# zhu-xlab/PFST

Measured on AMD Instinct MI355X. Metric: PFST train-step images/s on 1024² IRRG tiles, higher is better.
Workload: dtype f32 (f16x3 split MFMA: two scaled fp16 pieces per operand, three products, fp32 accumulate); 1 GPU; pfst_pots_irrg2vaih_irrg_deeplabv3plus_r50-d8; global_batch=8, per_gpu_batch=8, tile=1024x1024x3, num_classes=6, parallelism=dp1, weights=seeded random init, conv_math=f16x3

## Files before the change

### pfst_amd/csrc/conv_winograd.hip

```cpp
#include "common.h"
#include "amax.h"
#include "weight_jobs.h"

namespace {

template <int M> struct Wino;
template <> struct Wino<2> {
  static constexpr int R = 4;
  static constexpr float bt(int i, int j) {
    constexpr float m[4][4] = {{1, 0, -1, 0}, {0, 1, 1, 0}, {0, -1, 1, 0}, {0, 1, 0, -1}};
    return m[i][j];
  }
  static constexpr float g(int i, int j) {
    constexpr float m[4][3] = {{1, 0, 0}, {.5f, .5f, .5f}, {.5f, -.5f, .5f}, {0, 0, 1}};
    return m[i][j];
  }
  static constexpr float at(int i, int j) {
    constexpr float m[2][4] = {{1, 1, 1, 0}, {0, 1, -1, -1}};
    return m[i][j];
  }
};
template <> struct Wino<4> {
  static constexpr int R = 6;
  static constexpr float bt(int i, int j) {
    constexpr float m[6][6] = {{4, 0, -5, 0, 1, 0}, {0, -4, -4, 1, 1, 0}, {0, 4, -4, -1, 1, 0},
                               {0, -2, -1, 2, 1, 0}, {0, 2, -1, -2, 1, 0}, {0, 4, 0, -5, 0, 1}};
    return m[i][j];
  }
  static constexpr float g(int i, int j) {
    constexpr float m[6][3] = {{1.f / 4, 0, 0}, {-1.f / 6, -1.f / 6, -1.f / 6}, {-1.f / 6, 1.f / 6, -1.f / 6},
                               {1.f / 24, 1.f / 12, 1.f / 6}, {1.f / 24, -1.f / 12, 1.f / 6}, {0, 0, 1}};
    return m[i][j];
  }
  static constexpr float at(int i, int j) {
    constexpr float m[4][6] = {{1, 1, 1, 1, 1, 0}, {0, 1, -1, 2, -2, 0}, {0, 1, 1, 4, 4, 0}, {0, 1, -1, 8, -8, 1}};
    return m[i][j];
  }
};
__device__ __forceinline__ float cmac(float acc, float coef, float v) {
  if (coef == 0.f) return acc;
  if (coef == 1.f) return acc + v;
  if (coef == -1.f) return acc - v;
  return fmaf(coef, v, acc);
}

struct WinoGeom {
  int H, W, d, Hs, Ws, Th, Tw, T;
};
inline WinoGeom wino_geom(int H, int W, int d, int m) {
  WinoGeom g;
  g.H = H; g.W = W; g.d = d;
  g.Hs = (H + d - 1) / d; g.Ws = (W + d - 1) / d;
  g.Th = (g.Hs + m - 1) / m; g.Tw = (g.Ws + m - 1) / m;
  g.T = d * d * g.Th * g.Tw;
  return g;
}
__device__ __forceinline__ void tile_coord(const WinoGeom& g, int t, int& sy, int& sx, int& ty, int& tx) {
  sx = t % g.d; t /= g.d;
  tx = t % g.Tw; t /= g.Tw;
  ty = t % g.Th;
  sy = t / g.Th;
}

template <int M>
__device__ __forceinline__ void filter_tf(const float (&g)[3][3], float (&u)[M + 2][M + 2]) {
  constexpr int R = M + 2;
  float t[R][3];
#pragma unroll
  for (int i = 0; i < R; ++i)
#pragma unroll
    for (int j = 0; j < 3; ++j) {
      float a = 0.f;
#pragma unroll
      for (int k = 0; k < 3; ++k) a = cmac(a, Wino<M>::g(i, k), g[k][j]);
      t[i][j] = a;
    }
#pragma unroll
  for (int i = 0; i < R; ++i)
#pragma unroll
    for (int j = 0; j < R; ++j) {
      float a = 0.f;
#pragma unroll
      for (int k = 0; k < 3; ++k) a = cmac(a, Wino<M>::g(j, k), t[i][k]);
      u[i][j] = a;
    }
}
template <int M, bool PLAIN>
__global__ void wino_filter_kernel(const float* __restrict__ w, float* __restrict__ Uf, float* __restrict__ Ud, int Cout, int Cin) {
  constexpr int R = M + 2;
  const i64 total = (i64)Cout * Cin;
  for (i64 i = (i64)blockIdx.x * blockDim.x + threadIdx.x; i < total; i += (i64)gridDim.x * blockDim.x) {
    const int ci = (int)(i % Cin), co = (int)(i / Cin);
    float g[3][3], gf[3][3], u[R][R];
#pragma unroll
    for (int a = 0; a < 3; ++a)
#pragma unroll
      for (int b = 0; b < 3; ++b) {
        g[a][b] = w[i * 9 + a * 3 + b];
        gf[2 - a][2 - b] = g[a][b];
      }
    if (Uf) {
      filter_tf<M>(g, u);
      const i64 at = PLAIN ? i : ((i64)(ci >> 2) * Cout + co) * 4 + (ci & 3);
#pragma unroll
      for (int xi = 0; xi < R * R; ++xi) Uf[(i64)xi * total + at] = u[xi / R][xi % R];
    }
    if (Ud) {
      filter_tf<M>(gf, u);
      const i64 at = PLAIN ? i : ((i64)(co >> 2) * Cin + ci) * 4 + (co & 3);
#pragma unroll
      for (int xi = 0; xi < R * R; ++xi) Ud[(i64)xi * total + at] = u[xi / R][xi % R];
    }
  }
}

template <int M>
__global__ __launch_bounds__(256) void wino_input_kernel(const float* __restrict__ x, i64 x_bs, float* __restrict__ V, int N, int C,
                                                         WinoGeom g, int vec, float* __restrict__ amax, const float* __restrict__ pack_amax,
                                                         int pack_shift, const float4* __restrict__ bnl) {
  float am = 0.f;
  float ps = 0.f;
  if (pack_amax) {
    int e = amax_exponent(amax_read(pack_amax)) + pack_shift;
    e = e > 254 ? 254 : e;
    ps = scale_of(e);
    if (amax && blockIdx.x == 0 && blockIdx.y == 0 && blockIdx.z == 0 && threadIdx.x == 0) amax[0] = __builtin_bit_cast(float, (unsigned)e << 23);
  }
  constexpr int R = M + 2;
  typedef float vecM __attribute__((ext_vector_type(M)));
  const int c = blockIdx.y, n = blockIdx.z;
  const float* xp = x + (i64)n * x_bs + (i64)c * g.H * g.W;
  const i64 plane = (i64)N * C * g.T;
  float* vp = V + ((i64)n * C + c) * g.T;
  float nsc = 1.f, nsh = 0.f;
  if (bnl) {
    const float4 cf = bnl[c];
    nsc = cf.z;
    nsh = cf.w;
  }
  auto norm = [&](float v, bool in) { return bnl ? (in ? fmaxf(__fmaf_rn(v, nsc, nsh), 0.f) : 0.f) : v; };
  for (int t = blockIdx.x * blockDim.x + threadIdx.x; t < g.T; t += gridDim.x * blockDim.x) {
    int sy, sx, ty, tx;
    tile_coord(g, t, sy, sx, ty, tx);
    float d[R][R];
    if (vec) {
      const int x0 = M * tx;
#pragma unroll
      for (int a = 0; a < R; ++a) {
        const int y = M * ty - 1 + a;
        const bool in = y >= 0 && y < g.H;
        const float* row = xp + (i64)y * g.W + x0;
        vecM mid;
#pragma unroll
        for (int b = 0; b < M; ++b) mid[b] = 0.f;
        if (in) mid = *reinterpret_cast<const vecM*>(row);
        const bool inl = in && x0 > 0, inr = in && x0 + M < g.W;
        d[a][0] = norm(inl ? row[-1] : 0.f, inl);
#pragma unroll
        for (int b = 0; b < M; ++b) d[a][1 + b] = norm(mid[b], in);
        d[a][R - 1] = norm(inr ? row[M] : 0.f, inr);
      }
    } else {
#pragma unroll
      for (int a = 0; a < R; ++a) {
        const int y = sy + g.d * (M * ty - 1 + a);
#pragma unroll
        for (int b = 0; b < R; ++b) {
          const int xx = sx + g.d * (M * tx - 1 + b);
          const bool in = y >= 0 && y < g.H && xx >= 0 && xx < g.W;
          d[a][b] = norm(in ? xp[(i64)y * g.W + xx] : 0.f, in);
        }
      }
    }
    float r[R][R];
#pragma unroll
    for (int i = 0; i < R; ++i)
#pragma unroll
      for (int b = 0; b < R; ++b) {
        float a = 0.f;
#pragma unroll
        for (int k = 0; k < R; ++k) a = cmac(a, Wino<M>::bt(i, k), d[k][b]);
        r[i][b] = a;
      }
#pragma unroll
    for (int i = 0; i < R; ++i)
#pragma unroll
      for (int j = 0; j < R; ++j) {
        float a = 0.f;
#pragma unroll
        for (int k = 0; k < R; ++k) a = cmac(a, Wino<M>::bt(j, k), r[i][k]);
        if (pack_amax) {
          reinterpret_cast<unsigned*>(vp)[(i64)(i * R + j) * plane + t] = pack_f16x2_pieces(a * ps);
        } else {
          vp[(i64)(i * R + j) * plane + t] = a;
          am = fmaxf(am, fabsf(a));
        }
      }
  }
  if (amax && !pack_amax) amax_publish(amax, am);
}

template <int M>
__global__ __launch_bounds__(256) void wino_output_kernel(const float* __restrict__ Mb, float* __restrict__ y, i64 y_bs, int N, int Cout,
                                                          WinoGeom g, int accumulate, int vec, float* __restrict__ stats, int stats_minmax,
                                                          const float* __restrict__ bnb_x, i64 bnb_x_bs, const float4* __restrict__ bnb_coef, int bnb_relu) {
  constexpr int R = M + 2;
  typedef float vecM __attribute__((ext_vector_type(M)));
  __shared__ double red[32];
  float st_s = 0.f, st_q = 0.f;
  float st_lo = __builtin_inff(), st_hi = -__builtin_inff();
  const int c = blockIdx.y, n = blockIdx.z;
  float* yp = y + (i64)n * y_bs + (i64)c * g.H * g.W;
  const float* bxp = bnb_x ? bnb_x + (i64)n * bnb_x_bs + (i64)c * g.H * g.W : nullptr;
  const float bsc = bnb_x ? bnb_coef[c].z : 0.f, bsh = bnb_x ? bnb_coef[c].w : 0.f;
  const i64 plane = (i64)N * Cout * g.T;
  const float* mp = Mb + ((i64)n * Cout + c) * g.T;
  for (int t = blockIdx.x * blockDim.x + threadIdx.x; t < g.T; t += gridDim.x * blockDim.x) {
    int sy, sx, ty, tx;
    tile_coord(g, t, sy, sx, ty, tx);
    float m[R][R];
#pragma unroll
    for (int i = 0; i < R * R; ++i) m[i / R][i % R] = __builtin_nontemporal_load(&mp[(i64)i * plane + t]);
    float r[M][R];
#pragma unroll
    for (int i = 0; i < M; ++i)
#pragma unroll
      for (int b = 0; b < R; ++b) {
        float a = 0.f;
#pragma unroll
        for (int k = 0; k < R; ++k) a = cmac(a, Wino<M>::at(i, k), m[k][b]);
        r[i][b] = a;
      }
#pragma unroll
    for (int i = 0; i < M; ++i) {
      const int yy = sy + g.d * (M * ty + i);
      if (yy >= g.H) continue;
      float o[M];
#pragma unroll
      for (int j = 0; j < M; ++j) {
        float a = 0.f;
#pragma unroll
        for (int k = 0; k < R; ++k) a = cmac(a, Wino<M>::at(j, k), r[i][k]);
        o[j] = a;
      }
      const int x0 = sx + g.d * (M * tx);
      if (vec) {
        vecM* q = reinterpret_cast<vecM*>(yp + (i64)yy * g.W + x0);
        vecM v;
#pragma unroll
        for (int j = 0; j < M; ++j) v[j] = o[j];
        if (accumulate) v += *q;
        *q = v;
        if (bxp) {
          const vecM xv = *reinterpret_cast<const vecM*>(bxp + (i64)yy * g.W + x0);
#pragma unroll
          for (int j = 0; j < M; ++j) {
            const float dz = (!bnb_relu || __fmaf_rn(xv[j], bsc, bsh) > 0.f) ? v[j] : 0.f;
            st_s += dz;
            st_q = fmaf(dz, xv[j], st_q);
          }
          continue;
        }
#pragma unroll
        for (int j = 0; j < M; ++j) {
          const float e = v[j];
          st_s += e;
          st_q = fmaf(e, e, st_q);
          st_lo = fminf(st_lo, e);
          st_hi = fmaxf(st_hi, e);
        }
        continue;
      }
#pragma unroll
      for (int j = 0; j < M; ++j) {
        const int xx = x0 + g.d * j;
        if (xx < g.W) {
          float* q = yp + (i64)yy * g.W + xx;
          const float v = accumulate ? *q + o[j] : o[j];
          *q = v;
          if (bxp) {
            const float xs = bxp[(i64)yy * g.W + xx];
            const float dz = (!bnb_relu || __fmaf_rn(xs, bsc, bsh) > 0.f) ? v : 0.f;
            st_s += dz;
            st_q = fmaf(dz, xs, st_q);
          } else {
            st_s += v;
            st_q = fmaf(v, v, st_q);
            st_lo = fminf(st_lo, v);
            st_hi = fmaxf(st_hi, v);
          }
        }
      }
    }
  }
  if (stats) {
    double bs = (double)st_s, bq = (double)st_q;
    block_sum2_d<true>(bs, bq, red);
    if (threadIdx.x == 0) {
      const i64 T = (i64)gridDim.x * gridDim.z;
      float2* dst = reinterpret_cast<float2*>(stats) + ((i64)c * T + (i64)n * gridDim.x + blockIdx.x);
      *dst = make_float2((float)bs, (float)bq);
    }
    if (stats_minmax) {
#pragma unroll
      for (int o = 32; o > 0; o >>= 1) {
        st_lo = fminf(st_lo, __shfl_xor(st_lo, o));
        st_hi = fmaxf(st_hi, __shfl_xor(st_hi, o));
      }
      float* mm = reinterpret_cast<float*>(red);
      __syncthreads();
      if ((threadIdx.x & 63) == 0) { mm[threadIdx.x >> 6] = st_lo; mm[8 + (threadIdx.x >> 6)] = st_hi; }
      __syncthreads();
      if (threadIdx.x == 0) {
        const int nw = (blockDim.x + 63) >> 6;
        for (int i = 1; i < nw; ++i) { st_lo = fminf(st_lo, mm[i]); st_hi = fmaxf(st_hi, mm[8 + i]); }
        const i64 T = (i64)gridDim.x * gridDim.z;
        float2* dst = reinterpret_cast<float2*>(stats) + ((i64)Cout * T + (i64)c * T + (i64)n * gridDim.x + blockIdx.x);
        *dst = make_float2(st_lo, st_hi);
      }
    }
  }
}

template <int M>
__global__ __launch_bounds__(256) void wino_dy_kernel(const float* __restrict__ dy, i64 dy_bs, float* __restrict__ dM, int N, int Cout,
                                                      WinoGeom g, float* __restrict__ amax, const float* __restrict__ pack_amax, int pack_shift) {
  float am = 0.f;
  float ps = 0.f;
  if (pack_amax) {
    int e = amax_exponent(amax_read(pack_amax)) + pack_shift;
    e = e > 254 ? 254 : e;
    ps = scale_of(e);
    if (amax && blockIdx.x == 0 && blockIdx.y == 0 && blockIdx.z == 0 && threadIdx.x == 0) amax[0] = __builtin_bit_cast(float, (unsigned)e << 23);
  }
  constexpr int R = M + 2;
  const int c = blockIdx.y, n = blockIdx.z;
  const float* gp = dy + (i64)n * dy_bs + (i64)c * g.H * g.W;
  const i64 plane = (i64)N * Cout * g.T;
  float* mp = dM + ((i64)n * Cout + c) * g.T;
  for (int t = blockIdx.x * blockDim.x + threadIdx.x; t < g.T; t += gridDim.x * blockDim.x) {
    int sy, sx, ty, tx;
    tile_coord(g, t, sy, sx, ty, tx);
    float e[M][M];
#pragma unroll
    for (int i = 0; i < M; ++i)
#pragma unroll
      for (int j = 0; j < M; ++j) {
        const int yy = sy + g.d * (M * ty + i), xx = sx + g.d * (M * tx + j);
        e[i][j] = (yy < g.H && xx < g.W) ? gp[(i64)yy * g.W + xx] : 0.f;
      }
    float r[R][M];
#pragma unroll
    for (int a = 0; a < R; ++a)
#pragma unroll
      for (int j = 0; j < M; ++j) {
        float s = 0.f;
#pragma unroll
        for (int i = 0; i < M; ++i) s = cmac(s, Wino<M>::at(i, a), e[i][j]);
        r[a][j] = s;
      }
#pragma unroll
    for (int a = 0; a < R; ++a)
#pragma unroll
      for (int b = 0; b < R; ++b) {
        float s = 0.f;
#pragma unroll
        for (int j = 0; j < M; ++j) s = cmac(s, Wino<M>::at(j, b), r[a][j]);
        if (pack_amax) {
          reinterpret_cast<unsigned*>(mp)[(i64)(a * R + b) * plane + t] = pack_f16x2_pieces(s * ps);
        } else {
          mp[(i64)(a * R + b) * plane + t] = s;
          am = fmaxf(am, fabsf(s));
        }
      }
  }
  if (amax && !pack_amax) amax_publish(amax, am);
}

template <int M>
__global__ void wino_dw_kernel(const float* __restrict__ dU, float* __restrict__ dw, int Cout, int Cin) {
  constexpr int R = M + 2;
  const i64 total = (i64)Cout * Cin;
  for (i64 i = (i64)blockIdx.x * blockDim.x + threadIdx.x; i < total; i += (i64)gridDim.x * blockDim.x) {
    float u[R][R];
#pragma unroll
    for (int xi = 0; xi < R * R; ++xi) u[xi / R][xi % R] = dU[(i64)xi * total + i];
    float t[3][R];
#pragma unroll
    for (int p = 0; p < 3; ++p)
#pragma unroll
      for (int b = 0; b < R; ++b) {
        float s = 0.f;
#pragma unroll
        for (int a = 0; a < R; ++a) s = cmac(s, Wino<M>::g(a, p), u[a][b]);
        t[p][b] = s;
      }
#pragma unroll
    for (int p = 0; p < 3; ++p)
#pragma unroll
      for (int q = 0; q < 3; ++q) {
        float s = 0.f;
#pragma unroll
        for (int b = 0; b < R; ++b) s = cmac(s, Wino<M>::g(b, q), t[p][b]);
        dw[i * 9 + p * 3 + q] += s;
      }
  }
}

template <int M>
__device__ __forceinline__ void weight_prep_wino(const pfst_weight_job_t& J, int lb, float (*red)[36]) {
  constexpr int R = M + 2, X = R * R;
  const i64 total = (i64)J.Cout * J.Cin;
  const i64 i = (i64)lb * 256 + threadIdx.x;
  const bool live = i < total;
  float g[3][3], gf[3][3], u[R][R];
#pragma unroll
  for (int a = 0; a < 3; ++a)
#pragma unroll
    for (int b = 0; b < 3; ++b) {
      g[a][b] = live ? J.src[i * 9 + a * 3 + b] : 0.f;
      gf[2 - a][2 - b] = g[a][b];
    }
#pragma unroll
  for (int dir = 0; dir < 2; ++dir) {
    float* dst = reinterpret_cast<float*>(dir ? J.dst_d : J.dst_f);
    float* amax = dir ? J.amax_d : J.amax_f;
    if (!dst) continue;
    filter_tf<M>(dir ? gf : g, u);
#pragma unroll
    for (int xi = 0; xi < X; ++xi) {
      const float v = u[xi / R][xi % R];
      if (live) dst[(i64)xi * total + i] = v;
      float m = fabsf(v);
#pragma unroll
      for (int o = 32; o > 0; o >>= 1) m = fmaxf(m, __shfl_xor(m, o));
      if ((threadIdx.x & 63) == 0) red[threadIdx.x >> 6][xi] = m;
    }
    __syncthreads();
    if (threadIdx.x < X) {
      const float m = fmaxf(fmaxf(red[0][threadIdx.x], red[1][threadIdx.x]), fmaxf(red[2][threadIdx.x], red[3][threadIdx.x]));
      if (m > 0.f)
        atomicMax(reinterpret_cast<unsigned*>(amax) + (i64)threadIdx.x * PFST_AMAX_SUB + (lb & (PFST_AMAX_SUB - 1)), __builtin_bit_cast(unsigned, m));
    }
    __syncthreads();
  }
}

__global__ __launch_bounds__(256) void weight_prep_batched_kernel(const pfst_weight_job_t* __restrict__ jobs, int njobs) {
  __shared__ float red[4][36];
  const pfst_weight_job_t J = jobs[weight_job_of_block(jobs, njobs, blockIdx.x)];
  const int lb = blockIdx.x - J.first_block;
  if (J.m == 2) return weight_prep_wino<2>(J, lb, red);
  if (J.m == 4) return weight_prep_wino<4>(J, lb, red);
  const i64 n = (i64)J.Cout * J.Cin * J.T;
  float m = 0.f;
#pragma unroll 4
  for (int k = 0; k < 16; ++k) {
    const i64 i = (i64)lb * 4096 + k * 256 + threadIdx.x;
    if (i < n) m = fmaxf(m, fabsf(J.src[i]));
  }
#pragma unroll
  for (int o = 32; o > 0; o >>= 1) m = fmaxf(m, __shfl_xor(m, o));
  if ((threadIdx.x & 63) == 0) red[threadIdx.x >> 6][0] = m;
  __syncthreads();
  if (threadIdx.x == 0) {
    m = fmaxf(fmaxf(red[0][0], red[1][0]), fmaxf(red[2][0], red[3][0]));
    if (m > 0.f) atomicMax(reinterpret_cast<unsigned*>(J.amax_f) + (lb & (PFST_AMAX_SUB - 1)), __builtin_bit_cast(unsigned, m));
  }
}

inline int tile_blocks(int T) {
  int b = (T + 255) / 256;
  return b < 1 ? 1 : b;
}

#define PFST_WINO_M(m_, CALL2, CALL4) \
  do {                                \
    if ((m_) == 2) { CALL2; } else { CALL4; } \
  } while (0)

}

#define PFST_CHECK_TILE(m) PFST_CHECK_ARG((m) == 2 || (m) == 4)

extern "C" int pfst_wino_tiles(int H, int W, int dil, int m) {
  if (H <= 0 || W <= 0 || dil < 1 || (m != 2 && m != 4)) return 0;
  return wino_geom(H, W, dil, m).T;
}

extern "C" int pfst_wino_pack_weight(const float* w, float* U_fprop, float* U_dgrad, int Cout, int Cin, int m, pfst_stream_t stream) {
  PFST_CHECK_ARG(w && (U_fprop || U_dgrad) && Cout > 0 && Cin > 0);
  PFST_CHECK_TILE(m);
  PFST_CHECK_ARG((!U_fprop || Cin % 16 == 0) && (!U_dgrad || Cout % 16 == 0));
  const dim3 grid(ew_grid((i64)Cout * Cin));
  PFST_WINO_M(m, hipLaunchKernelGGL((wino_filter_kernel<2, false>), grid, dim3(256), 0, (hipStream_t)stream, w, U_fprop, U_dgrad, Cout, Cin),
              hipLaunchKernelGGL((wino_filter_kernel<4, false>), grid, dim3(256), 0, (hipStream_t)stream, w, U_fprop, U_dgrad, Cout, Cin));
  PFST_CHECK_LAUNCH();
  return PFST_OK;
}

extern "C" int pfst_wino_filter_plain(const float* w, float* P_fprop, float* P_dgrad, int Cout, int Cin, int m, pfst_stream_t stream) {
  PFST_CHECK_ARG(w && (P_fprop || P_dgrad) && Cout > 0 && Cin > 0);
  PFST_CHECK_TILE(m);
  const dim3 grid(ew_grid((i64)Cout * Cin));
  PFST_WINO_M(m, hipLaunchKernelGGL((wino_filter_kernel<2, true>), grid, dim3(256), 0, (hipStream_t)stream, w, P_fprop, P_dgrad, Cout, Cin),
              hipLaunchKernelGGL((wino_filter_kernel<4, true>), grid, dim3(256), 0, (hipStream_t)stream, w, P_fprop, P_dgrad, Cout, Cin));
  PFST_CHECK_LAUNCH();
  return PFST_OK;
}

extern "C" int pfst_weight_job_blocks(const pfst_weight_job_t* job, int pack) { return job ? weight_job_blocks(*job, pack) : 0; }

extern "C" int pfst_weight_prep_batched(const pfst_weight_job_t* jobs_host, const pfst_weight_job_t* jobs_dev, int njobs, pfst_stream_t stream) {
  PFST_CHECK_ARG(jobs_host && jobs_dev && njobs > 0);
  i64 blocks = 0;
  for (int j = 0; j < njobs; ++j) {
    const pfst_weight_job_t& J = jobs_host[j];
    PFST_CHECK_ARG(J.src && J.Cout > 0 && J.Cin > 0 && (J.m == 0 || J.m == 2 || J.m == 4) && J.first_block == blocks);
    if (J.m == 0) PFST_CHECK_ARG(J.amax_f && (J.T == 1 || J.T == 9));
    else PFST_CHECK_ARG(J.T == 9 && (J.dst_f || J.dst_d) && (!J.dst_f || J.amax_f) && (!J.dst_d || J.amax_d));
    blocks += weight_job_blocks(J, 0);
  }
  PFST_CHECK_ARG(blocks < (1ll << 31));
  hipLaunchKernelGGL(weight_prep_batched_kernel, dim3((unsigned)blocks), dim3(256), 0, (hipStream_t)stream, jobs_dev, njobs);
  PFST_CHECK_LAUNCH();
  return PFST_OK;
}

extern "C" int pfst_wino_input(const float* x, long long x_bs, float* V, int N, int C, int H, int W, int dil, int m, float* v_amax,
                               const float* pack_x_amax, const float* bnl, pfst_stream_t stream) {
  PFST_CHECK_ARG(!pack_x_amax || v_amax);
  PFST_CHECK_ARG(!bnl || ((uintptr_t)bnl & 15) == 0);
  const int shift_in = m == 4 ? 7 : 3;
  PFST_CHECK_ARG(x && V && N > 0 && N <= 65535 && C > 0 && C <= 65535 && H > 0 && W > 0 && dil >= 1 && x_bs >= (i64)C * H * W);
  PFST_CHECK_TILE(m);
  const WinoGeom g = wino_geom(H, W, dil, m);
  const int vec = dil == 1 && W % m == 0 && x_bs % m == 0 && ((uintptr_t)x & (4 * m - 1)) == 0;
  const dim3 grid(tile_blocks(g.T), C, N);
  PFST_WINO_M(m, hipLaunchKernelGGL(wino_input_kernel<2>, grid, dim3(256), 0, (hipStream_t)stream, x, x_bs, V, N, C, g, vec, v_amax, pack_x_amax, shift_in, (const float4*)bnl),
              hipLaunchKernelGGL(wino_input_kernel<4>, grid, dim3(256), 0, (hipStream_t)stream, x, x_bs, V, N, C, g, vec, v_amax, pack_x_amax, shift_in, (const float4*)bnl));
  PFST_CHECK_LAUNCH();
  return PFST_OK;
}

extern "C" int pfst_wino_gemm(const float* V, const float* U, float* Mbuf, int N, int K, int M, int T, int m, pfst_stream_t stream) {
  PFST_CHECK_ARG(V && U && Mbuf && N > 0 && N <= 65535 && K > 0 && K % 16 == 0 && M > 0 && T > 0);
  PFST_CHECK_TILE(m);
  PFST_CHECK_ARG((i64)K * T * 4 < (1ll << 31) && (i64)M * T * 4 < (1ll << 31) && (i64)K * M * 4 < (1ll << 31));
  return pfst_igemm_q_launch(V, (i64)K * T, U, nullptr, Mbuf, (i64)M * T, N, K, 1, T, M, 1, T, 1, 1, 1, 0, 1, 0, nullptr, 0,
                             (m + 2) * (m + 2), (hipStream_t)stream);
}

extern "C" int pfst_wino_stats_slots(int H, int W, int dil, int m) {
  if (H <= 0 || W <= 0 || dil < 1 || (m != 2 && m != 4)) return 0;
  return tile_blocks(wino_geom(H, W, dil, m).T);
}

extern "C" int pfst_wino_output(const float* Mbuf, float* y, long long y_bs, int N, int Cout, int H, int W, int dil, int accumulate,
                                float* stats, int stats_minmax, const float* bnb_x, long long bnb_x_bs, const float* bnb_coef, int bnb_relu, int m,
                                pfst_stream_t stream) {
  PFST_CHECK_ARG(Mbuf && y && N > 0 && N <= 65535 && Cout > 0 && Cout <= 65535 && H > 0 && W > 0 && dil >= 1 && y_bs >= (i64)Cout * H * W);
  PFST_CHECK_ARG(!stats_minmax || stats);
  PFST_CHECK_ARG(!bnb_x || (stats && !stats_minmax && bnb_coef && bnb_x_bs >= (i64)Cout * H * W && (bnb_x_bs % 4) == 0 && ((uintptr_t)bnb_x & 15) == 0));
  PFST_CHECK_TILE(m);
  const WinoGeom g = wino_geom(H, W, dil, m);
  const int vec = dil == 1 && W % m == 0 && y_bs % m == 0 && ((uintptr_t)y & (4 * m - 1)) == 0;
  const dim3 grid(tile_blocks(g.T), Cout, N);
  PFST_WINO_M(m, hipLaunchKernelGGL(wino_output_kernel<2>, grid, dim3(256), 0, (hipStream_t)stream, Mbuf, y, y_bs, N, Cout, g, accumulate, vec, stats, stats_minmax, bnb_x,
                                 (i64)bnb_x_bs, reinterpret_cast<const float4*>(bnb_coef), bnb_relu),
              hipLaunchKernelGGL(wino_output_kernel<4>, grid, dim3(256), 0, (hipStream_t)stream, Mbuf, y, y_bs, N, Cout, g, accumulate, vec, stats, stats_minmax, bnb_x,
                                 (i64)bnb_x_bs, reinterpret_cast<const float4*>(bnb_coef), bnb_relu));
  PFST_CHECK_LAUNCH();
  return PFST_OK;
}

extern "C" int pfst_wino_dy(const float* dy, long long dy_bs, float* dM, int N, int Cout, int H, int W, int dil, int m, float* dm_amax,
                            const float* pack_dy_amax, pfst_stream_t stream) {
  PFST_CHECK_ARG(!pack_dy_amax || dm_amax);
  const int shift_dy = m == 4 ? 8 : 2;
  PFST_CHECK_ARG(dy && dM && N > 0 && N <= 65535 && Cout > 0 && Cout <= 65535 && H > 0 && W > 0 && dil >= 1 && dy_bs >= (i64)Cout * H * W);
  PFST_CHECK_TILE(m);
  const WinoGeom g = wino_geom(H, W, dil, m);
  const dim3 grid(tile_blocks(g.T), Cout, N);
  PFST_WINO_M(m, hipLaunchKernelGGL(wino_dy_kernel<2>, grid, dim3(256), 0, (hipStream_t)stream, dy, dy_bs, dM, N, Cout, g, dm_amax, pack_dy_amax, shift_dy),
              hipLaunchKernelGGL(wino_dy_kernel<4>, grid, dim3(256), 0, (hipStream_t)stream, dy, dy_bs, dM, N, Cout, g, dm_amax, pack_dy_amax, shift_dy));
  PFST_CHECK_LAUNCH();
  return PFST_OK;
}

extern "C" int pfst_wino_wgrad(const float* V, const float* dM, float* dU, float* dw, int N, int Cin, int Cout, int T, int m,
                               int split, const float* v_amax, const float* dm_amax, int packed, pfst_stream_t stream) {
  PFST_CHECK_ARG(V && dM && dU && dw && N > 0 && N <= 65535 && Cin > 0 && Cout > 0 && T > 0 && T % 4 == 0);
  PFST_CHECK_ARG(split != 2 || (v_amax && dm_amax && Cout > 64));
  PFST_CHECK_ARG(!packed || split == 2);
  PFST_CHECK_TILE(m);
  hipStream_t s = (hipStream_t)stream;
  const i64 uc = (i64)Cout * Cin;
  const int nx = (m + 2) * (m + 2);
  if (hipMemsetAsync(dU, 0, nx * uc * sizeof(float), s) != hipSuccess) return PFST_ERR_LAUNCH;
  const int rc = split == 2 ? pfst_wgrad_f16x3_launch(V, (i64)Cin * T, dM, (i64)Cout * T, dU, N, Cin, Cout, T, nx, (i64)N * Cin * T,
                                                      (i64)N * Cout * T, uc, v_amax, dm_amax, packed, s)
                 : split ? pfst_wgrad_split_q_launch(V, (i64)Cin * T, dM, (i64)Cout * T, dU, N, Cin, Cout, T, nx, (i64)N * Cin * T,
                                                   (i64)N * Cout * T, uc, s)
                       : pfst_wgrad_q_launch(V, (i64)Cin * T, dM, (i64)Cout * T, dU, N, Cin, 1, T, Cout, 1, T, 1, 1, 0, nx, (i64)N * Cin * T,
                                             (i64)N * Cout * T, uc, s);
  if (rc != PFST_OK) return rc;
  PFST_WINO_M(m, hipLaunchKernelGGL(wino_dw_kernel<2>, dim3(ew_grid(uc)), dim3(256), 0, s, dU, dw, Cout, Cin),
              hipLaunchKernelGGL(wino_dw_kernel<4>, dim3(ew_grid(uc)), dim3(256), 0, s, dU, dw, Cout, Cin));
  PFST_CHECK_LAUNCH();
  return PFST_OK;
}
```

Baseline: 29.59 images/s.

## Stage Winograd input/dy/output row bands through LDS with coalesced vector loads

Adds an LDS staging path for the Winograd input, dy and output transform kernels. Each 256-thread block loads or stores its contiguous band of image rows with coalesced float4 accesses into padded shared memory, where wino_pos adds bank-conflict padding. Tiles are then read from or written to LDS instead of through strided global gathers, which matters most for dilated convolutions. The cost is up to 63KB of dynamic LDS per block, which can lower occupancy, plus extra barriers and more template variants. The path can be disabled with the PFST_WINO_STAGED environment variable, and the output kernel uses it only when dilation is greater than 1.

Measured after the change: 29.83 images/s (median of 6 runs). About the same (+0.8%).

```diff
diff --git a/pfst_amd/csrc/conv_winograd.hip b/pfst_amd/csrc/conv_winograd.hip
--- a/pfst_amd/csrc/conv_winograd.hip
+++ b/pfst_amd/csrc/conv_winograd.hip
@@ -1,3 +1,4 @@
+#include <stdlib.h>
 #include "common.h"
 #include "amax.h"
 #include "weight_jobs.h"
@@ -62,6 +63,105 @@
   sy = t / g.Th;
 }
 
+typedef float f4 __attribute__((ext_vector_type(4)));
+constexpr int kWinoStageBudget = 63 * 1024;
+struct WinoStage {
+  int on, LP, XE, P, rows;
+};
+__host__ __device__ __forceinline__ int wino_pos(int x, int d) { return x + d * (x >> 5); }
+inline WinoStage wino_stage(const WinoGeom& g, int m, int halo, int images, bool aligned, unsigned& bytes) {
+  WinoStage st = {0, 0, 0, 0, 0};
+  bytes = 0;
+  const char* e = getenv("PFST_WINO_STAGED");
+  if ((e && e[0] == '0' && !e[1]) || !aligned || g.W % 4 != 0 || (halo && g.d > 4)) return st;
+  const i64 L = (i64)g.Tw * g.d;
+  i64 nty = 256 % L == 0 ? 256 / L : 254 / L + 2;
+  nty = nty > g.Th ? g.Th : nty;
+  st.LP = halo ? 4 : 0;
+  st.XE = g.d * m * g.Tw + (halo ? g.d : 0);
+  st.P = (wino_pos(st.LP + st.XE - 1, g.d) + 1) | 1;
+  st.rows = (int)(m * nty + 2 * halo);
+  const i64 need = (i64)images * st.rows * st.P * 4;
+  if (need > kWinoStageBudget) return st;
+  bytes = (unsigned)need;
+  st.on = 1;
+  return st;
+}
+__device__ __forceinline__ int div_u(int a, int b, float rb) {
+  int q = (int)((float)a * rb);
+  const int r = a - q * b;
+  q += (r >= b) - (r < 0);
+  return q;
+}
+struct WinoBand {
+  int ok, sy, ty0, nty, tbase, L;
+  float rL, rd;
+};
+__device__ __forceinline__ WinoBand wino_band(const WinoGeom& g, const WinoStage& st, int m, int halo) {
+  WinoBand b;
+  const int t0 = blockIdx.x * 256, t1 = min(t0 + 255, g.T - 1);
+  int sx, tx, sy1, ty1;
+  tile_coord(g, t0, b.sy, sx, b.ty0, tx);
+  tile_coord(g, t1, sy1, sx, ty1, tx);
+  b.nty = ty1 - b.ty0 + 1;
+  b.L = g.Tw * g.d;
+  b.tbase = (b.sy * g.Th + b.ty0) * b.L;
+  b.ok = st.on && sy1 == b.sy && m * b.nty + 2 * halo <= st.rows;
+  b.rL = 1.f / (float)b.L;
+  b.rd = 1.f / (float)g.d;
+  return b;
+}
+__device__ __forceinline__ void band_coord(const WinoGeom& g, const WinoBand& b, int t, int& tyr, int& sx, int& tx) {
+  const int rel = t - b.tbase;
+  tyr = div_u(rel, b.L, b.rL);
+  const int rem = rel - tyr * b.L;
+  tx = div_u(rem, g.d, b.rd);
+  sx = rem - tx * g.d;
+}
+template <bool PADS, bool NT>
+__device__ __forceinline__ void stage_rows(float* __restrict__ lds, const float* __restrict__ src, const WinoGeom& g, const WinoStage& st, int sy,
+                                           int r0, int NR, bool norm, float nsc, float nsh) {
+  const int W4 = g.W >> 2, n4 = NR * W4;
+  const float rW4 = 1.f / (float)W4;
+  constexpr int U = 6;
+  for (int i0 = threadIdx.x; i0 < n4; i0 += 256 * U) {
+    f4 v[U];
+    int at[U];
+    bool in[U];
+#pragma unroll
+    for (int u = 0; u < U; ++u) {
+      const int i = i0 + 256 * u;
+      at[u] = -1;
+      in[u] = false;
+      v[u] = (f4)(0.f);
+      if (i < n4) {
+        const int rr = div_u(i, W4, rW4), c4 = i - rr * W4;
+        const int y = sy + g.d * (r0 + rr);
+        at[u] = rr * st.P + wino_pos(st.LP + 4 * c4, g.d);
+        in[u] = y >= 0 && y < g.H;
+        if (in[u]) {
+          const f4* q = reinterpret_cast<const f4*>(src + (i64)y * g.W) + c4;
+          v[u] = NT ? __builtin_nontemporal_load(q) : *q;
+        }
+      }
+    }
+#pragma unroll
+    for (int u = 0; u < U; ++u)
+      if (at[u] >= 0) {
+#pragma unroll
+        for (int k = 0; k < 4; ++k) lds[at[u] + k] = (norm && in[u]) ? fmaxf(__fmaf_rn(v[u][k], nsc, nsh), 0.f) : v[u][k];
+      }
+  }
+  if (PADS) {
+    const int np = st.LP + st.XE - g.W;
+    const float rnp = 1.f / (float)np;
+    for (int i = threadIdx.x; i < NR * np; i += 256) {
+      const int rr = div_u(i, np, rnp), k = i - rr * np;
+      lds[rr * st.P + wino_pos(k < st.LP ? k : g.W + k, g.d)] = 0.f;
+    }
+  }
+}
+
 template <int M>
 __device__ __forceinline__ void filter_tf(const float (&g)[3][3], float (&u)[M + 2][M + 2]) {
   constexpr int R = M + 2;
@@ -114,10 +214,11 @@
   }
 }
 
-template <int M>
+extern __shared__ float wino_lds[];
+template <int M, bool ST>
 __global__ __launch_bounds__(256) void wino_input_kernel(const float* __restrict__ x, i64 x_bs, float* __restrict__ V, int N, int C,
                                                          WinoGeom g, int vec, float* __restrict__ amax, const float* __restrict__ pack_amax,
-                                                         int pack_shift, const float4* __restrict__ bnl) {
+                                                         int pack_shift, const float4* __restrict__ bnl, WinoStage st) {
   float am = 0.f;
   float ps = 0.f;
   if (pack_amax) {
@@ -139,11 +240,30 @@
     nsh = cf.w;
   }
   auto norm = [&](float v, bool in) { return bnl ? (in ? fmaxf(__fmaf_rn(v, nsc, nsh), 0.f) : 0.f) : v; };
+  WinoBand bd;
+  bd.ok = 0;
+  if (ST) {
+    bd = wino_band(g, st, M, 1);
+    if (bd.ok) {
+      stage_rows<true, true>(wino_lds, xp, g, st, bd.sy, M * bd.ty0 - 1, M * bd.nty + 2, bnl != nullptr, nsc, nsh);
+      __syncthreads();
+    }
+  }
   for (int t = blockIdx.x * blockDim.x + threadIdx.x; t < g.T; t += gridDim.x * blockDim.x) {
     int sy, sx, ty, tx;
-    tile_coord(g, t, sy, sx, ty, tx);
+    if (!(ST && bd.ok)) tile_coord(g, t, sy, sx, ty, tx);
     float d[R][R];
-    if (vec) {
+    if (ST && bd.ok) {
+      band_coord(g, bd, t, ty, sx, tx);
+      const float* row = wino_lds + M * ty * st.P;
+      int cp[R];
+#pragma unroll
+      for (int b = 0; b < R; ++b) cp[b] = wino_pos(st.LP + sx + g.d * (M * tx - 1 + b), g.d);
+#pragma unroll
+      for (int a = 0; a < R; ++a)
+#pragma unroll
+        for (int b = 0; b < R; ++b) d[a][b] = row[a * st.P + cp[b]];
+    } else if (vec) {
       const int x0 = M * tx;
 #pragma unroll
       for (int a = 0; a < R; ++a) {
@@ -200,10 +320,11 @@
   if (amax && !pack_amax) amax_publish(amax, am);
 }
 
-template <int M>
+template <int M, bool ST>
 __global__ __launch_bounds__(256) void wino_output_kernel(const float* __restrict__ Mb, float* __restrict__ y, i64 y_bs, int N, int Cout,
                                                           WinoGeom g, int accumulate, int vec, float* __restrict__ stats, int stats_minmax,
-                                                          const float* __restrict__ bnb_x, i64 bnb_x_bs, const float4* __restrict__ bnb_coef, int bnb_relu) {
+                                                          const float* __restrict__ bnb_x, i64 bnb_x_bs, const float4* __restrict__ bnb_coef, int bnb_relu,
+                                                          WinoStage st) {
   constexpr int R = M + 2;
   typedef float vecM __attribute__((ext_vector_type(M)));
   __shared__ double red[32];
@@ -215,6 +336,122 @@
   const float bsc = bnb_x ? bnb_coef[c].z : 0.f, bsh = bnb_x ? bnb_coef[c].w : 0.f;
   const i64 plane = (i64)N * Cout * g.T;
   const float* mp = Mb + ((i64)n * Cout + c) * g.T;
+  WinoBand bd;
+  bd.ok = 0;
+  if (ST) bd = wino_band(g, st, M, 0);
+  if (ST && bd.ok) {
+    float* yimg = wino_lds;
+    float* ximg = (bxp && accumulate) ? wino_lds + st.rows * st.P : wino_lds;
+    const int NR = M * bd.nty, r0 = M * bd.ty0;
+    const int t = blockIdx.x * 256 + threadIdx.x;
+    const bool live = t < g.T;
+    int ty = 0, sx = 0, tx = 0;
+    float v[M][M];
+    int cp[M];
+    if (live) {
+      band_coord(g, bd, t, ty, sx, tx);
+#pragma unroll
+      for (int j = 0; j < M; ++j) cp[j] = M * ty * st.P + wino_pos(sx + g.d * (M * tx + j), g.d);
+      float m[R][R];
+#pragma unroll
+      for (int i = 0; i < R * R; ++i) m[i / R][i % R] = __builtin_nontemporal_load(&mp[(i64)i * plane + t]);
+      float r[M][R];
+#pragma unroll
+      for (int i = 0; i < M; ++i)
+#pragma unroll
+        for (int b = 0; b < R; ++b) {
+          float a = 0.f;
+#pragma unroll
+          for (int k = 0; k < R; ++k) a = cmac(a, Wino<M>::at(i, k), m[k][b]);
+          r[i][b] = a;
+        }
+#pragma unroll
+      for (int i = 0; i < M; ++i)
+#pragma unroll
+        for (int j = 0; j < M; ++j) {
+          float a = 0.f;
+#pragma unroll
+          for (int k = 0; k < R; ++k) a = cmac(a, Wino<M>::at(j, k), r[i][k]);
+          v[i][j] = a;
+          yimg[i * st.P + cp[j]] = a;
+        }
+    }
+    auto sums = [&]() {
+      if (live) {
+#pragma unroll
+        for (int i = 0; i < M; ++i) {
+          if (bd.sy + g.d * (r0 + M * ty + i) >= g.H) continue;
+#pragma unroll
+          for (int j = 0; j < M; ++j) {
+            if (sx + g.d * (M * tx + j) >= g.W) continue;
+            const float e = accumulate ? yimg[i * st.P + cp[j]] : v[i][j];
+            if (bxp) {
+              const float xs = ximg[i * st.P + cp[j]];
+              const float dz = (!bnb_relu || __fmaf_rn(xs, bsc, bsh) > 0.f) ? e : 0.f;
+              st_s += dz;
+              st_q = fmaf(dz, xs, st_q);
+            } else {
+              st_s += e;
+              st_q = fmaf(e, e, st_q);
+              st_lo = fminf(st_lo, e);
+              st_hi = fmaxf(st_hi, e);
+            }
+          }
+        }
+      }
+    };
+    const bool late = accumulate || bxp;
+    if (stats && !late) sums();
+    __syncthreads();
+    {
+      const int W4 = g.W >> 2, n4 = NR * W4;
+      const float rW4 = 1.f / (float)W4;
+      constexpr int U = 2;
+      for (int i0 = threadIdx.x; i0 < n4; i0 += 256 * U) {
+        f4 old[U], bx[U];
+        int at[U];
+        f4* dst[U];
+#pragma unroll
+        for (int u = 0; u < U; ++u) {
+          const int i = i0 + 256 * u;
+          at[u] = -1;
+          old[u] = (f4)(0.f);
+          bx[u] = (f4)(0.f);
+          if (i < n4) {
+            const int rr = div_u(i, W4, rW4), c4 = i - rr * W4;
+            const int yy = bd.sy + g.d * (r0 + rr);
+            if (yy < g.H) {
+              at[u] = rr * st.P + wino_pos(4 * c4, g.d);
+              dst[u] = reinterpret_cast<f4*>(yp + (i64)yy * g.W) + c4;
+              if (accumulate) old[u] = *dst[u];
+              if (bxp) bx[u] = *(reinterpret_cast<const f4*>(bxp + (i64)yy * g.W) + c4);
+            }
+          }
+        }
+#pragma unroll
+        for (int u = 0; u < U; ++u)
+          if (at[u] >= 0) {
+            f4 w;
+#pragma unroll
+            for (int k = 0; k < 4; ++k) w[k] = yimg[at[u] + k];
+            if (accumulate) w = old[u] + w;
+            *dst[u] = w;
+            if (stats && accumulate) {
+#pragma unroll
+              for (int k = 0; k < 4; ++k) yimg[at[u] + k] = w[k];
+            }
+            if (bxp) {
+#pragma unroll
+              for (int k = 0; k < 4; ++k) ximg[at[u] + k] = bx[u][k];
+            }
+          }
+      }
+    }
+    if (stats && late) {
+      __syncthreads();
+      sums();
+    }
+  } else
   for (int t = blockIdx.x * blockDim.x + threadIdx.x; t < g.T; t += gridDim.x * blockDim.x) {
     int sy, sx, ty, tx;
     tile_coord(g, t, sy, sx, ty, tx);
@@ -322,9 +559,10 @@
   }
 }
 
-template <int M>
+template <int M, bool ST>
 __global__ __launch_bounds__(256) void wino_dy_kernel(const float* __restrict__ dy, i64 dy_bs, float* __restrict__ dM, int N, int Cout,
-                                                      WinoGeom g, float* __restrict__ amax, const float* __restrict__ pack_amax, int pack_shift) {
+                                                      WinoGeom g, float* __restrict__ amax, const float* __restrict__ pack_amax, int pack_shift,
+                                                      WinoStage st) {
   float am = 0.f;
   float ps = 0.f;
   if (pack_amax) {
@@ -338,17 +576,38 @@
   const float* gp = dy + (i64)n * dy_bs + (i64)c * g.H * g.W;
   const i64 plane = (i64)N * Cout * g.T;
   float* mp = dM + ((i64)n * Cout + c) * g.T;
+  WinoBand bd;
+  bd.ok = 0;
+  if (ST) {
+    bd = wino_band(g, st, M, 0);
+    if (bd.ok) {
+      stage_rows<true, true>(wino_lds, gp, g, st, bd.sy, M * bd.ty0, M * bd.nty, false, 1.f, 0.f);
+      __syncthreads();
+    }
+  }
   for (int t = blockIdx.x * blockDim.x + threadIdx.x; t < g.T; t += gridDim.x * blockDim.x) {
     int sy, sx, ty, tx;
-    tile_coord(g, t, sy, sx, ty, tx);
     float e[M][M];
-#pragma unroll
-    for (int i = 0; i < M; ++i)
-#pragma unroll
-      for (int j = 0; j < M; ++j) {
-        const int yy = sy + g.d * (M * ty + i), xx = sx + g.d * (M * tx + j);
-        e[i][j] = (yy < g.H && xx < g.W) ? gp[(i64)yy * g.W + xx] : 0.f;
-      }
+    if (ST && bd.ok) {
+      band_coord(g, bd, t, ty, sx, tx);
+      const float* row = wino_lds + M * ty * st.P;
+      int cp[M];
+#pragma unroll
+      for (int j = 0; j < M; ++j) cp[j] = wino_pos(sx + g.d * (M * tx + j), g.d);
+#pragma unroll
+      for (int i = 0; i < M; ++i)
+#pragma unroll
+        for (int j = 0; j < M; ++j) e[i][j] = row[i * st.P + cp[j]];
+    } else {
+      tile_coord(g, t, sy, sx, ty, tx);
+#pragma unroll
+      for (int i = 0; i < M; ++i)
+#pragma unroll
+        for (int j = 0; j < M; ++j) {
+          const int yy = sy + g.d * (M * ty + i), xx = sx + g.d * (M * tx + j);
+          e[i][j] = (yy < g.H && xx < g.W) ? gp[(i64)yy * g.W + xx] : 0.f;
+        }
+    }
     float r[R][M];
 #pragma unroll
     for (int a = 0; a < R; ++a)
@@ -537,8 +796,13 @@
   const WinoGeom g = wino_geom(H, W, dil, m);
   const int vec = dil == 1 && W % m == 0 && x_bs % m == 0 && ((uintptr_t)x & (4 * m - 1)) == 0;
   const dim3 grid(tile_blocks(g.T), C, N);
-  PFST_WINO_M(m, hipLaunchKernelGGL(wino_input_kernel<2>, grid, dim3(256), 0, (hipStream_t)stream, x, x_bs, V, N, C, g, vec, v_amax, pack_x_amax, shift_in, (const float4*)bnl),
-              hipLaunchKernelGGL(wino_input_kernel<4>, grid, dim3(256), 0, (hipStream_t)stream, x, x_bs, V, N, C, g, vec, v_amax, pack_x_amax, shift_in, (const float4*)bnl));
+  unsigned lds;
+  const WinoStage st = wino_stage(g, m, 1, 1, x_bs % 4 == 0 && ((uintptr_t)x & 15) == 0, lds);
+#define PFST_WINO_INPUT(M_, ST_) \
+  hipLaunchKernelGGL((wino_input_kernel<M_, ST_>), grid, dim3(256), lds, (hipStream_t)stream, x, x_bs, V, N, C, g, vec, v_amax, pack_x_amax, shift_in, (const float4*)bnl, st)
+  if (st.on) PFST_WINO_M(m, PFST_WINO_INPUT(2, true), PFST_WINO_INPUT(4, true));
+  else PFST_WINO_M(m, PFST_WINO_INPUT(2, false), PFST_WINO_INPUT(4, false));
+#undef PFST_WINO_INPUT
   PFST_CHECK_LAUNCH();
   return PFST_OK;
 }
@@ -566,10 +830,14 @@
   const WinoGeom g = wino_geom(H, W, dil, m);
   const int vec = dil == 1 && W % m == 0 && y_bs % m == 0 && ((uintptr_t)y & (4 * m - 1)) == 0;
   const dim3 grid(tile_blocks(g.T), Cout, N);
-  PFST_WINO_M(m, hipLaunchKernelGGL(wino_output_kernel<2>, grid, dim3(256), 0, (hipStream_t)stream, Mbuf, y, y_bs, N, Cout, g, accumulate, vec, stats, stats_minmax, bnb_x,
-                                 (i64)bnb_x_bs, reinterpret_cast<const float4*>(bnb_coef), bnb_relu),
-              hipLaunchKernelGGL(wino_output_kernel<4>, grid, dim3(256), 0, (hipStream_t)stream, Mbuf, y, y_bs, N, Cout, g, accumulate, vec, stats, stats_minmax, bnb_x,
-                                 (i64)bnb_x_bs, reinterpret_cast<const float4*>(bnb_coef), bnb_relu));
+  unsigned lds;
+  const WinoStage st = wino_stage(g, m, 0, bnb_x && accumulate ? 2 : 1, dil > 1 && y_bs % 4 == 0 && ((uintptr_t)y & 15) == 0, lds);
+#define PFST_WINO_OUTPUT(M_, ST_)                                                                                                                                  \
+  hipLaunchKernelGGL((wino_output_kernel<M_, ST_>), grid, dim3(256), lds, (hipStream_t)stream, Mbuf, y, y_bs, N, Cout, g, accumulate, vec, stats, stats_minmax, bnb_x, \
+                     (i64)bnb_x_bs, reinterpret_cast<const float4*>(bnb_coef), bnb_relu, st)
+  if (st.on) PFST_WINO_M(m, PFST_WINO_OUTPUT(2, true), PFST_WINO_OUTPUT(4, true));
+  else PFST_WINO_M(m, PFST_WINO_OUTPUT(2, false), PFST_WINO_OUTPUT(4, false));
+#undef PFST_WINO_OUTPUT
   PFST_CHECK_LAUNCH();
   return PFST_OK;
 }
@@ -582,8 +850,13 @@
   PFST_CHECK_TILE(m);
   const WinoGeom g = wino_geom(H, W, dil, m);
   const dim3 grid(tile_blocks(g.T), Cout, N);
-  PFST_WINO_M(m, hipLaunchKernelGGL(wino_dy_kernel<2>, grid, dim3(256), 0, (hipStream_t)stream, dy, dy_bs, dM, N, Cout, g, dm_amax, pack_dy_amax, shift_dy),
-              hipLaunchKernelGGL(wino_dy_kernel<4>, grid, dim3(256), 0, (hipStream_t)stream, dy, dy_bs, dM, N, Cout, g, dm_amax, pack_dy_amax, shift_dy));
+  unsigned lds;
+  const WinoStage st = wino_stage(g, m, 0, 1, dy_bs % 4 == 0 && ((uintptr_t)dy & 15) == 0, lds);
+#define PFST_WINO_DY(M_, ST_) \
+  hipLaunchKernelGGL((wino_dy_kernel<M_, ST_>), grid, dim3(256), lds, (hipStream_t)stream, dy, dy_bs, dM, N, Cout, g, dm_amax, pack_dy_amax, shift_dy, st)
+  if (st.on) PFST_WINO_M(m, PFST_WINO_DY(2, true), PFST_WINO_DY(4, true));
+  else PFST_WINO_M(m, PFST_WINO_DY(2, false), PFST_WINO_DY(4, false));
+#undef PFST_WINO_DY
   PFST_CHECK_LAUNCH();
   return PFST_OK;
 }
```
